# boundless-xyz/boundless

Hardware: AMD Instinct MI355X
Metric: segment-proofs/sec @ 2^20 cycles (higher is better)
Workload: dtype u32 (BabyBear Montgomery)

## Files before the change

### boundless_amd/csrc/poseidon2.hip

```cpp
#include "ctx.hpp"
#include "poseidon2_arith.hpp"
#include "hash_suite.hpp"
#include "../../include/bx_image.h"

namespace bx {

constexpr int CELLS = 24, RATE = 16, RF_HALF = 4, RP = 21;
constexpr int DIAG_OFF = 216;

__device__ __forceinline__ void poseidon2_mix(uint32_t* io, const uint32_t* __restrict__ prm) {
    i32 s[CELLS];
    i64 y[CELLS];
#pragma unroll
    for (int i = 0; i < CELLS; ++i) s[i] = (i32)io[i];
    m_ext64s(s, y);
    redc64s_all(y, prm, s);
#pragma unroll 1
    for (int r = 0; r < RF_HALF; ++r) {
        sbox7s_n<CELLS / 2>(s);
        sbox7s_n<CELLS / 2>(s + CELLS / 2);
        m_ext64s(s, y);
        if (r < RF_HALF - 1) {
            redc64s_all(y, prm + (r + 1) * CELLS, s);
        } else {
            red64ks_all<K1_MID, K2_MID, true>(y, prm[96], s);
        }
    }
    uint32_t diag[CELLS];
    {
        uint32_t zero;
        asm volatile("v_mov_b32 %0, 0" : "=v"(zero));
        const uint4* dp = reinterpret_cast<const uint4*>(prm + DIAG_OFF + zero);
#pragma unroll
        for (int i = 0; i < CELLS / 4; ++i) {
            const uint4 v = dp[i];
            diag[4 * i] = __builtin_amdgcn_readfirstlane(v.x);
            diag[4 * i + 1] = __builtin_amdgcn_readfirstlane(v.y);
            diag[4 * i + 2] = __builtin_amdgcn_readfirstlane(v.z);
            diag[4 * i + 3] = __builtin_amdgcn_readfirstlane(v.w);
        }
    }
#pragma unroll 1
    for (int r = 0; r < RP - 1; ++r) {
        internal_round<false>(s, diag, prm + 97 + r);
    }
    internal_round<true>(s, diag, prm + 117);
#pragma unroll 1
    for (int r = 0; r < RF_HALF; ++r) {
        sbox7s_n<CELLS / 2>(s);
        sbox7s_n<CELLS / 2>(s + CELLS / 2);
        m_ext64s(s, y);
        if (r < RF_HALF - 1) {
            redc64s_all(y, prm + 117 + (r + 1) * CELLS, s);
        } else {
            red64ks_all<K1_END, K2_END, false>(y, 0u, s);
#pragma unroll
            for (int i = 0; i < CELLS; ++i) io[i] = canon(s[i]);
        }
    }
}

__global__ __launch_bounds__(256) __attribute__((amdgpu_waves_per_eu(4, 4))) void hash_rows_kernel(uint32_t* __restrict__ out, const uint32_t* __restrict__ matrix,
                                                        const uint32_t* __restrict__ prm, uint32_t rows, uint32_t cols) {
    uint32_t r = blockIdx.x * blockDim.x + threadIdx.x;
    if (r >= rows) return;
    uint32_t s[CELLS];
#pragma unroll
    for (int i = 0; i < CELLS; ++i) s[i] = 0u;
    const uint32_t* p = matrix + r;
    uint32_t c = 0;
    for (; c + RATE <= cols; c += RATE) {
#pragma unroll
        for (int i = 0; i < RATE; ++i) s[i] = p[(size_t)(c + i) * rows];
        poseidon2_mix(s, prm);
    }
    if (c < cols || cols == 0) {
#pragma unroll
        for (int i = 0; i < RATE; ++i) s[i] = (c + i < cols) ? p[(size_t)(c + i) * rows] : 0u;
        poseidon2_mix(s, prm);
    }
    uint4* o = reinterpret_cast<uint4*>(out + (size_t)r * 8);
    o[0] = make_uint4(s[0], s[1], s[2], s[3]);
    o[1] = make_uint4(s[4], s[5], s[6], s[7]);
}

__global__ __launch_bounds__(256) __attribute__((amdgpu_waves_per_eu(4, 4))) void hash_fold_kernel(uint32_t* __restrict__ io, const uint32_t* __restrict__ prm,
                                                        uint32_t input_size, uint32_t output_size) {
    uint32_t i = blockIdx.x * blockDim.x + threadIdx.x;
    if (i >= output_size) return;
    const uint4* src = reinterpret_cast<const uint4*>(io + ((size_t)input_size + 2 * (size_t)i) * 8);
    uint32_t s[CELLS];
    uint4 v0 = src[0], v1 = src[1], v2 = src[2], v3 = src[3];
    s[0] = v0.x; s[1] = v0.y; s[2] = v0.z; s[3] = v0.w;
    s[4] = v1.x; s[5] = v1.y; s[6] = v1.z; s[7] = v1.w;
    s[8] = v2.x; s[9] = v2.y; s[10] = v2.z; s[11] = v2.w;
    s[12] = v3.x; s[13] = v3.y; s[14] = v3.z; s[15] = v3.w;
#pragma unroll
    for (int k = 16; k < CELLS; ++k) s[k] = 0u;
    poseidon2_mix(s, prm);
    uint4* o = reinterpret_cast<uint4*>(io + ((size_t)output_size + i) * 8);
    o[0] = make_uint4(s[0], s[1], s[2], s[3]);
    o[1] = make_uint4(s[4], s[5], s[6], s[7]);
}

__global__ __launch_bounds__(256) __attribute__((amdgpu_waves_per_eu(4, 4))) void hash_fold_indexed_kernel(uint32_t* out, const uint32_t* in,
                                                                const uint32_t* __restrict__ sel, const uint32_t* __restrict__ prm,
                                                                uint32_t count, uint32_t n_in) {
    uint32_t j = blockIdx.x * blockDim.x + threadIdx.x;
    if (j >= count) return;
    uint2 pr = reinterpret_cast<const uint2*>(sel)[j];
    pr.x = pr.x < n_in ? pr.x : n_in - 1;
    pr.y = pr.y < n_in ? pr.y : n_in - 1;
    const uint4* a = reinterpret_cast<const uint4*>(in + (size_t)pr.x * 8);
    const uint4* b = reinterpret_cast<const uint4*>(in + (size_t)pr.y * 8);
    uint32_t s[CELLS];
    uint4 v0 = a[0], v1 = a[1], v2 = b[0], v3 = b[1];
    s[0] = v0.x; s[1] = v0.y; s[2] = v0.z; s[3] = v0.w;
    s[4] = v1.x; s[5] = v1.y; s[6] = v1.z; s[7] = v1.w;
    s[8] = v2.x; s[9] = v2.y; s[10] = v2.z; s[11] = v2.w;
    s[12] = v3.x; s[13] = v3.y; s[14] = v3.z; s[15] = v3.w;
#pragma unroll
    for (int k = 16; k < CELLS; ++k) s[k] = 0u;
    poseidon2_mix(s, prm);
    uint4* o = reinterpret_cast<uint4*>(out + (size_t)j * 8);
    o[0] = make_uint4(s[0], s[1], s[2], s[3]);
    o[1] = make_uint4(s[4], s[5], s[6], s[7]);
}

__device__ __forceinline__ void fold_pair(uint32_t* out8, const uint32_t* a8, const uint32_t* b8, const uint32_t* __restrict__ prm) {
    uint32_t s[CELLS];
#pragma unroll
    for (int k = 0; k < 8; ++k) s[k] = a8[k], s[8 + k] = b8[k];
#pragma unroll
    for (int k = 16; k < CELLS; ++k) s[k] = 0u;
    poseidon2_mix(s, prm);
#pragma unroll
    for (int k = 0; k < 8; ++k) out8[k] = s[k];
}
__device__ __forceinline__ void ld_digest(uint32_t* d, const uint32_t* p) {
    const uint4 a = reinterpret_cast<const uint4*>(p)[0], b = reinterpret_cast<const uint4*>(p)[1];
    d[0] = a.x; d[1] = a.y; d[2] = a.z; d[3] = a.w; d[4] = b.x; d[5] = b.y; d[6] = b.z; d[7] = b.w;
}
__device__ __forceinline__ void st_digest(uint32_t* p, const uint32_t* d) {
    reinterpret_cast<uint4*>(p)[0] = make_uint4(d[0], d[1], d[2], d[3]);
    reinterpret_cast<uint4*>(p)[1] = make_uint4(d[4], d[5], d[6], d[7]);
}
template <int LVL>
__device__ __forceinline__ void fold_subtree(uint32_t* out8, uint32_t* __restrict__ io, const uint32_t* __restrict__ prm, size_t input_size, size_t idx) {
    uint32_t a[8], b[8];
    if constexpr (LVL == 1) {
        ld_digest(a, io + (input_size + 2 * idx) * 8);
        ld_digest(b, io + (input_size + 2 * idx + 1) * 8);
    } else {
        fold_subtree<LVL - 1>(a, io, prm, input_size, 2 * idx);
        fold_subtree<LVL - 1>(b, io, prm, input_size, 2 * idx + 1);
    }
    fold_pair(out8, a, b, prm);
    st_digest(io + ((input_size >> LVL) + idx) * 8, out8);
}
template <int L>
__global__ __launch_bounds__(256) __attribute__((amdgpu_waves_per_eu(4, 4))) void hash_fold_deep_kernel(uint32_t* __restrict__ io, const uint32_t* __restrict__ prm,
                                                                                               uint32_t input_size) {
    const uint32_t j = blockIdx.x * blockDim.x + threadIdx.x;
    if (j >= (input_size >> L)) return;
    uint32_t top[8];
    fold_subtree<L>(top, io, prm, input_size, j);
}

__global__ __launch_bounds__(256) __attribute__((amdgpu_waves_per_eu(4, 4))) void hash_fold_multi_kernel(uint32_t* __restrict__ io, const uint32_t* __restrict__ prm,
                                                              uint32_t input_size, uint32_t per_wg, int levels) {
    __shared__ uint32_t sh[256 * 8];
    const uint32_t tid = threadIdx.x;
    uint32_t width = per_wg >> 1;
    uint32_t out_size = input_size >> 1;
    uint32_t s[CELLS];
    if (tid < width) {
        const uint32_t i = blockIdx.x * width + tid;
        const uint4* src = reinterpret_cast<const uint4*>(io + ((size_t)input_size + 2 * (size_t)i) * 8);
        uint4 v0 = src[0], v1 = src[1], v2 = src[2], v3 = src[3];
        s[0] = v0.x; s[1] = v0.y; s[2] = v0.z; s[3] = v0.w;
        s[4] = v1.x; s[5] = v1.y; s[6] = v1.z; s[7] = v1.w;
        s[8] = v2.x; s[9] = v2.y; s[10] = v2.z; s[11] = v2.w;
        s[12] = v3.x; s[13] = v3.y; s[14] = v3.z; s[15] = v3.w;
#pragma unroll
        for (int k = 16; k < CELLS; ++k) s[k] = 0u;
        poseidon2_mix(s, prm);
        uint4* o = reinterpret_cast<uint4*>(io + ((size_t)out_size + i) * 8);
        o[0] = make_uint4(s[0], s[1], s[2], s[3]);
        o[1] = make_uint4(s[4], s[5], s[6], s[7]);
    }
    for (int lvl = 1; lvl < levels; ++lvl) {
        if (tid < width) {
#pragma unroll
            for (int k = 0; k < 8; ++k) sh[tid * 8 + k] = s[k];
        }
        __syncthreads();
        width >>= 1;
        out_size >>= 1;
        if (tid < width) {
#pragma unroll
            for (int k = 0; k < 16; ++k) s[k] = sh[tid * 16 + k];
#pragma unroll
            for (int k = 16; k < CELLS; ++k) s[k] = 0u;
            poseidon2_mix(s, prm);
            uint4* o = reinterpret_cast<uint4*>(io + ((size_t)out_size + blockIdx.x * width + tid) * 8);
            o[0] = make_uint4(s[0], s[1], s[2], s[3]);
            o[1] = make_uint4(s[4], s[5], s[6], s[7]);
        }
        __syncthreads();
    }
}

constexpr int QS = CELLS / 4;
__device__ __forceinline__ i32 quad_rot1(i32 v) { return __builtin_amdgcn_update_dpp(0, v, 0x39, 0xf, 0xf, false); }
__device__ __forceinline__ i32 quad_rot2(i32 v) { return __builtin_amdgcn_update_dpp(0, v, 0x4E, 0xf, 0xf, false); }
__device__ __forceinline__ i32 quad_rot3(i32 v) { return __builtin_amdgcn_update_dpp(0, v, 0x93, 0xf, 0xf, false); }
__device__ __forceinline__ i32 quad_xor1(i32 v) { return __builtin_amdgcn_update_dpp(0, v, 0xB1, 0xf, 0xf, false); }
__device__ __forceinline__ i64 add_u32v(i64 c, uint32_t k, int alt) {
#if defined(__HIP_DEVICE_COMPILE__)
    i64 r;
    BX_MAD_ASM("v_mad_u64_u32", "%1, 1, %2", "v"(k), "v"(c));
    return r;
#else
    (void)alt;
    return c + (i64)k;
#endif
}
struct QuadCoef {
    i32 c0, c1, c3;
};
__device__ __forceinline__ void m_ext_quad(const i32* s, i64* y, const QuadCoef& m) {
    i64 t = 0;
#pragma unroll
    for (int k = 0; k < QS; ++k) {
        const i32 x1 = quad_rot1(s[k]), x2 = quad_rot2(s[k]), x3 = quad_rot3(s[k]);
        i64 w = smul(s[k], m.c0, k);
        w = smad(x1, m.c1, w, k + 1);
        w = smadc<1>(x2, w, k + 2);
        w = smad(x3, m.c3, w, k + 3);
        y[k] = w;
        t += w;
    }
#pragma unroll
    for (int k = 0; k < QS; ++k) y[k] += t;
}
__device__ __forceinline__ void redc_quad(const i64* y, const uint32_t* __restrict__ rc , i32* s) {
    i64 acc[QS];
#pragma unroll
    for (int k = 0; k < QS; ++k) acc[k] = add_u32v(y[k], rc[4 * k], k);
    sredc_n<QS>(acc, s);
}
template <uint32_t K1, uint32_t K2>
__device__ __forceinline__ void redk_quad(const i64* y, uint32_t add0 , i32* s) {
    i64 acc[QS];
#pragma unroll
    for (int k = 0; k < QS; ++k) acc[k] = umul_k((uint32_t)y[k], K1, k);
    acc[0] = add_u32v(acc[0], add0, 0);
#pragma unroll
    for (int k = 0; k < QS; ++k) acc[k] = smad_k((i32)(y[k] >> 32), K2, acc[k], k + 1);
    sredc_n<QS>(acc, s);
}
template <bool RC_ALL>
__device__ __forceinline__ void internal_round_quad(i32* s, const i32* diag, uint32_t rc0 ,
                                                    const uint32_t* __restrict__ rc_all, uint32_t keep_mask) {
    const i32 sb = sbox7s(s[0]);
    s[0] = (i32)(((uint32_t)sb & keep_mask) | ((uint32_t)s[0] & ~keep_mask));
    i64 pa = smulc<1>(s[0], 0);
#pragma unroll
    for (int k = 1; k < QS; ++k) pa = smadc<1>(s[k], pa, k);
    {
        i64 o = (i64)(((uint64_t)(uint32_t)quad_xor1((i32)(pa >> 32)) << 32) | (uint32_t)quad_xor1((i32)(uint32_t)pa));
        pa += o;
        o = (i64)(((uint64_t)(uint32_t)quad_rot2((i32)(pa >> 32)) << 32) | (uint32_t)quad_rot2((i32)(uint32_t)pa));
        pa += o;
    }
    const i64 c = smulc<1>(internal_sum_rs(pa), 1);
    i64 tt[QS];
#pragma unroll
    for (int k = 0; k < QS; ++k) {
        if (RC_ALL) tt[k] = smad(s[k], diag[k], add_u32v(c, rc_all[4 * k], 2 * k), 2 * k + 1);
        else if (k == 0) tt[k] = smad(s[k], diag[k], add_u32v(c, rc0, 0), 1);
        else tt[k] = smad(s[k], diag[k], c, k + 1);
    }
    sredc_n<QS>(tt, s);
}
__device__ __forceinline__ void poseidon2_mix_quad(uint32_t* io, const uint32_t* __restrict__ shp, uint32_t q) {
    i32 s[QS];
    i64 y[QS];
    const bool odd = q & 1;
    const QuadCoef m{odd ? 6 : 5, odd ? 1 : 7, odd ? 4 : 3};
    const uint32_t keep = q == 0 ? 0xffffffffu : 0u;
#pragma unroll
    for (int k = 0; k < QS; ++k) s[k] = (i32)io[k];
    m_ext_quad(s, y, m);
    redc_quad(y, shp + q, s);
#pragma unroll 1
    for (int r = 0; r < RF_HALF; ++r) {
        sbox7s_n<QS>(s);
        m_ext_quad(s, y, m);
        if (r < RF_HALF - 1) redc_quad(y, shp + (r + 1) * CELLS + q, s);
        else redk_quad<K1_MID, K2_MID>(y, shp[96] & keep, s);
    }
    i32 diag[QS];
#pragma unroll
    for (int k = 0; k < QS; ++k) diag[k] = (i32)shp[DIAG_OFF + 4 * k + q];
#pragma unroll 1
    for (int r = 0; r < RP - 1; ++r) internal_round_quad<false>(s, diag, shp[97 + r] & keep, nullptr, keep);
    internal_round_quad<true>(s, diag, 0u, shp + 117 + q, keep);
#pragma unroll 1
    for (int r = 0; r < RF_HALF; ++r) {
        sbox7s_n<QS>(s);
        m_ext_quad(s, y, m);
        if (r < RF_HALF - 1) redc_quad(y, shp + 117 + (r + 1) * CELLS + q, s);
        else redk_quad<K1_END, K2_END>(y, 0u, s);
    }
#pragma unroll
    for (int k = 0; k < QS; ++k) io[k] = canon(s[k]);
}

__global__ __launch_bounds__(1024) void hash_fold_quad_kernel(uint32_t* __restrict__ io, const uint32_t* __restrict__ prm, uint32_t input_size,
                                                              uint32_t per_wg, int levels) {
    __shared__ uint32_t sh[256 * 8];
    __shared__ uint32_t shp[DIAG_OFF + 24];
    const uint32_t tid = threadIdx.x, q = tid & 3, node = tid >> 2;
    for (uint32_t i = tid; i < DIAG_OFF + 24; i += blockDim.x) shp[i] = prm[i];
    uint32_t width = per_wg >> 1;
    uint32_t out_size = input_size >> 1;
    for (int lvl = 0; lvl < levels; ++lvl) {
        const bool active = node < width;
        uint32_t s[QS];
        if (active) {
            if (lvl == 0) {
                const uint32_t* src = io + ((size_t)input_size + 2 * ((size_t)blockIdx.x * width + node)) * 8;
#pragma unroll
                for (int k = 0; k < 4; ++k) s[k] = src[4 * k + q];
            } else {
#pragma unroll
                for (int k = 0; k < 4; ++k) s[k] = sh[node * 16 + 4 * k + q];
            }
            s[4] = 0u;
            s[5] = 0u;
        }
        __syncthreads();
        if (active) {
            poseidon2_mix_quad(s, shp, q);
            uint32_t* o = io + ((size_t)out_size + (size_t)blockIdx.x * width + node) * 8;
            o[q] = s[0];
            o[4 + q] = s[1];
            sh[node * 8 + q] = s[0];
            sh[node * 8 + 4 + q] = s[1];
        }
        __syncthreads();
        width >>= 1;
        out_size >>= 1;
    }
}

__global__ __launch_bounds__(64) void transcript_step_kernel(uint32_t* __restrict__ state, const uint32_t* __restrict__ digests, uint32_t n_commit,
                                                            uint32_t* __restrict__ out, uint32_t n_elems, const uint32_t* __restrict__ prm) {
    __shared__ uint32_t shp[DIAG_OFF + 24];
    const uint32_t tid = threadIdx.x, q = tid & 3;
    for (uint32_t i = tid; i < DIAG_OFF + 24; i += blockDim.x) shp[i] = prm[i];
    __syncthreads();
    if (tid >= 4) return;
    uint32_t s[QS];
#pragma unroll
    for (int k = 0; k < QS; ++k) s[k] = state[4 * k + q];
    uint32_t pool = state[24];
    for (uint32_t i = 0; i < n_commit; ++i) {
        if (pool != 0) {
            poseidon2_mix_quad(s, shp, q);
            pool = 0;
        }
        s[0] = fp_add(s[0], digests[8 * i + q]);
        s[1] = fp_add(s[1], digests[8 * i + 4 + q]);
        poseidon2_mix_quad(s, shp, q);
    }
    for (uint32_t e = 0; e < n_elems; ++e) {
        if (pool == 16) {
            poseidon2_mix_quad(s, shp, q);
            pool = 0;
        }
        const uint32_t slot = pool >> 2;
        const uint32_t v = slot == 0 ? s[0] : slot == 1 ? s[1] : slot == 2 ? s[2] : s[3];
        if ((pool & 3u) == q) out[e] = v;
        ++pool;
    }
#pragma unroll
    for (int k = 0; k < QS; ++k) state[4 * k + q] = s[k];
    if (q == 0) state[24] = pool;
}

const char* poseidon2_upload_params(bx_ctx* c) {
    uint32_t h[DIAG_OFF + 24] = {0};
    for (int i = 0; i < 213; ++i) h[i] = (uint32_t)((uint64_t)(c->h_rc[i] % P) * p2_rc_scale(i) % P);
    for (int i = 0; i < 24; ++i) h[DIAG_OFF + i] = fp_encode(c->h_diag[i]);
    if (!c->d_p2) BX_HIP(c, hipMalloc(&c->d_p2, sizeof h));
    BX_HIP(c, hipMemcpyAsync(c->d_p2, h, sizeof h, hipMemcpyHostToDevice, c->stream));
    BX_HIP(c, stream_wait(c));
    return nullptr;
}

static const char* launch_hash_rows(bx_ctx* c, uint32_t* out, const uint32_t* matrix, size_t rows, size_t cols) {
    if (rows == 0) return nullptr;
    unsigned bs = (unsigned)c->hash_rows_block;
    hipLaunchKernelGGL(hash_rows_kernel, dim3((unsigned)((rows + bs - 1) / bs)), dim3(bs), 0, c->stream, out, matrix, c->d_p2,
                       (uint32_t)rows, (uint32_t)cols);
    BX_LAUNCH_CHECK(c);
    return nullptr;
}
static const char* launch_hash_fold(bx_ctx* c, uint32_t* io, size_t input_size, size_t output_size) {
    if (output_size == 0) return nullptr;
    hipLaunchKernelGGL(hash_fold_kernel, dim3((unsigned)((output_size + 255) / 256)), dim3(256), 0, c->stream, io, c->d_p2,
                       (uint32_t)input_size, (uint32_t)output_size);
    BX_LAUNCH_CHECK(c);
    return nullptr;
}
template <int L>
static const char* launch_hash_fold_deep(bx_ctx* c, uint32_t* io, size_t size) {
    hipLaunchKernelGGL(hash_fold_deep_kernel<L>, dim3((unsigned)(((size >> L) + 255) / 256)), dim3(256), 0, c->stream, io, c->d_p2, (uint32_t)size);
    BX_LAUNCH_CHECK(c);
    return nullptr;
}
static const char* launch_hash_fold_small(bx_ctx* c, uint32_t* io, size_t size, size_t per_wg, int levels) {
    if (c->fold_quad)
        hipLaunchKernelGGL(hash_fold_quad_kernel, dim3((unsigned)(size / per_wg)), dim3((unsigned)(2 * per_wg)), 0, c->stream, io, c->d_p2,
                           (uint32_t)size, (uint32_t)per_wg, levels);
    else
        hipLaunchKernelGGL(hash_fold_multi_kernel, dim3((unsigned)(size / per_wg)), dim3(256), 0, c->stream, io, c->d_p2, (uint32_t)size,
                           (uint32_t)per_wg, levels);
    BX_LAUNCH_CHECK(c);
    return nullptr;
}
HashLaunchers poseidon2_launchers() { return {launch_hash_rows, launch_hash_fold, launch_hash_fold_deep<3>, launch_hash_fold_deep<2>, launch_hash_fold_small}; }

}

using namespace bx;

extern "C" const char* bx_poseidon2_set_params(bx_ctx* c, const uint32_t* rc213, const uint32_t* diag24) try {
    if (!c) return "bx_poseidon2_set_params: null ctx";
    BX_REQUIRE(c, rc213 && diag24, "poseidon2_set_params: null table");
    BX_REQUIRE(c, c->live_provers == 0, "poseidon2_set_params: destroy the provers of this ctx first (their transcripts hold the old table)");
    BX_ENTER(c);
    for (int i = 0; i < 213; ++i) c->h_rc[i] = rc213[i] % P;
    for (int i = 0; i < 24; ++i) c->h_diag[i] = diag24[i] % P;
    return poseidon2_upload_params(c);
} BX_ABI_CATCH(c, "bx_poseidon2_set_params")
extern "C" const char* bx_poseidon2_get_params(bx_ctx* c, uint32_t* rc213, uint32_t* diag24) try {
    if (!c) return "bx_poseidon2_get_params: null ctx";
    for (int i = 0; i < 213; ++i) rc213[i] = c->h_rc[i];
    for (int i = 0; i < 24; ++i) diag24[i] = c->h_diag[i];
    return nullptr;
} BX_ABI_CATCH(c, "bx_poseidon2_get_params")

extern "C" const char* bx_hash_fold_indexed(bx_ctx* c, bx_buf out, bx_buf in, bx_buf sel, size_t count) try {
    if (!c) return "bx_hash_fold_indexed: null ctx";
    BX_REQUIRE(c, count <= out.len / 8 && count <= sel.len / 2, "hash_fold_indexed: out or sel too small");
    BX_REQUIRE(c, count <= 0xffffffffu && in.len / 8 <= 0xffffffffu, "hash_fold_indexed: too many digests");
    if (count == 0) return nullptr;
    BX_REQUIRE(c, out.dptr && in.dptr && sel.dptr && in.len >= 8, "hash_fold_indexed: null or empty buffer");
    BX_ENTER(c);
    OpScope op(c, "hash_fold_indexed", 104.0 * (double)count);
    hipLaunchKernelGGL(hash_fold_indexed_kernel, dim3((unsigned)((count + 255) / 256)), dim3(256), 0, c->stream, (uint32_t*)out.dptr,
                       (const uint32_t*)in.dptr, (const uint32_t*)sel.dptr, c->d_p2, (uint32_t)count, (uint32_t)(in.len / 8));
    BX_LAUNCH_CHECK(c);
    return nullptr;
} BX_ABI_CATCH(c, "bx_hash_fold_indexed")

extern "C" const char* bx_transcript_step(bx_ctx* c, bx_buf state, bx_buf digests, size_t n_commit, bx_buf out_ext, size_t n_ext) try {
    if (!c) return "bx_transcript_step: null ctx";
    BX_REQUIRE(c, c->hash_suite == SUITE_POSEIDON2, "transcript_step: the device transcript is Poseidon2's (a sha-256 ctx draws on the host)");
    BX_REQUIRE(c, state.dptr != nullptr && state.len >= 25, "transcript_step: the state is 24 cells and the pool counter");
    BX_REQUIRE(c, n_commit <= 64 && n_ext <= 64, "transcript_step: at most 64 commits and 64 challenges per step");
    BX_REQUIRE(c, digests.len >= 8 * n_commit && out_ext.len >= 4 * n_ext, "transcript_step: digests / out too small");
    BX_ENTER(c);
    if (!n_commit && !n_ext) return nullptr;
    OpScope op(c, "transcript_step", 4.0 * (double)(50 + 8 * n_commit + 4 * n_ext));
    hipLaunchKernelGGL(transcript_step_kernel, dim3(1), dim3(64), 0, c->stream, (uint32_t*)state.dptr, (const uint32_t*)digests.dptr, (uint32_t)n_commit,
                       (uint32_t*)out_ext.dptr, (uint32_t)(4 * n_ext), c->d_p2);
    BX_LAUNCH_CHECK(c);
    return nullptr;
} BX_ABI_CATCH(c, "bx_transcript_step")
```

### boundless_amd/csrc/poseidon2_arith.hpp

```cpp
#pragma once
#include "fp.hpp"

#if defined(BX_CHECK_BOUNDS) && !defined(__HIP_DEVICE_COMPILE__)
#include <stdio.h>
#include <stdlib.h>
#define BX_ASSERT_BOUND(cond, what)                                              \
    do {                                                                         \
        if (!(cond)) {                                                           \
            fprintf(stderr, "bound violated: %s (%s:%d)\n", what, __FILE__, __LINE__); \
            abort();                                                             \
        }                                                                        \
    } while (0)
#else
#define BX_ASSERT_BOUND(cond, what) ((void)0)
#endif

#if defined(BX_PLAIN_MAD)
#define BX_MAD_FLAVOUR mad_plain
#else
#define BX_MAD_FLAVOUR mad_pinned
#endif
namespace bx {
inline namespace BX_MAD_FLAVOUR {

constexpr int P2_CELLS = 24;

constexpr uint32_t cx_mul(uint32_t a, uint32_t b) { return (uint32_t)((uint64_t)a * b % P); }
constexpr uint32_t cx_pow(uint32_t b, uint64_t e) {
    uint32_t r = 1;
    while (e) {
        if (e & 1) r = cx_mul(r, b);
        b = cx_mul(b, b);
        e >>= 1;
    }
    return r;
}
constexpr uint32_t cx_rpow(int64_t e) { return cx_pow(MONT_ONE, e >= 0 ? (uint64_t)e : (uint64_t)((int64_t)(P - 1) + e)); }
constexpr uint32_t K1_MID = cx_rpow(2801), K2_MID = cx_mul(K1_MID, MONT_ONE);
constexpr uint32_t K1_END = cx_rpow(400), K2_END = cx_mul(K1_END, MONT_ONE);
constexpr uint32_t p2_rc_scale(int i) {
    return i < 24 ? cx_rpow(1) : i < 48 ? cx_rpow(-6) : i < 72 ? cx_rpow(-55) : i < 96 ? cx_rpow(-398)
         : i < 141 ? cx_rpow(2)
         : i < 165 ? cx_rpow(1) : i < 189 ? cx_rpow(-6) : cx_rpow(-55);
}

using i32 = int32_t;
using i64 = int64_t;
constexpr i64 SREDC_MAX = ((i64)0x7fffffff - (i64)(P / 2) - 2) * ((i64)1 << 32);

#if defined(__HIP_DEVICE_COMPILE__) && !defined(BX_PLAIN_MAD)
#define BX_MAD_ASM(op, args, ...)                                                                  \
    do {                                                                                           \
        switch (alt & 3) {                                                                         \
            case 0: asm volatile(op " %0, s[40:41], " args : "=v"(r) : __VA_ARGS__ : "s40", "s41"); break; \
            case 1: asm volatile(op " %0, s[42:43], " args : "=v"(r) : __VA_ARGS__ : "s42", "s43"); break; \
            case 2: asm volatile(op " %0, s[44:45], " args : "=v"(r) : __VA_ARGS__ : "s44", "s45"); break; \
            default: asm volatile(op " %0, s[46:47], " args : "=v"(r) : __VA_ARGS__ : "s46", "s47"); break; \
        }                                                                                          \
    } while (0)
#endif
BX_HD i64 smad(i32 a, i32 b, i64 c, int alt = 0) {
#if defined(__HIP_DEVICE_COMPILE__) && !defined(BX_PLAIN_MAD)
    i64 r;
    BX_MAD_ASM("v_mad_i64_i32", "%1, %2, %3", "v"(a), "v"(b), "v"(c));
    return r;
#else
    (void)alt;
    return (i64)a * (i64)b + c;
#endif
}
BX_HD i64 smul(i32 a, i32 b, int alt = 0) {
#if defined(__HIP_DEVICE_COMPILE__) && !defined(BX_PLAIN_MAD)
    i64 r;
    BX_MAD_ASM("v_mad_i64_i32", "%1, %2, 0", "v"(a), "v"(b));
    return r;
#else
    (void)alt;
    return (i64)a * (i64)b;
#endif
}
BX_HD i64 smad_k(i32 a, uint32_t k, i64 c, int alt = 0) {
#if defined(__HIP_DEVICE_COMPILE__) && !defined(BX_PLAIN_MAD)
    i64 r;
    BX_MAD_ASM("v_mad_i64_i32", "%1, %2, %3", "v"(a), "s"(k), "v"(c));
    return r;
#else
    (void)alt;
    return (i64)a * (i64)k + c;
#endif
}
BX_HD i64 smul_k(i32 a, uint32_t k, int alt = 0) {
#if defined(__HIP_DEVICE_COMPILE__) && !defined(BX_PLAIN_MAD)
    i64 r;
    BX_MAD_ASM("v_mad_i64_i32", "%1, %2, 0", "v"(a), "s"(k));
    return r;
#else
    (void)alt;
    return (i64)a * (i64)k;
#endif
}
template <int K>
BX_HD i64 smadc(i32 a, i64 c, int alt = 0) {
#if defined(__HIP_DEVICE_COMPILE__) && !defined(BX_PLAIN_MAD)
    i64 r;
    BX_MAD_ASM("v_mad_i64_i32", "%1, %3, %2", "v"(a), "v"(c), "n"(K));
    return r;
#else
    (void)alt;
    return (i64)a * K + c;
#endif
}
template <int K>
BX_HD i64 smulc(i32 a, int alt = 0) {
#if defined(__HIP_DEVICE_COMPILE__) && !defined(BX_PLAIN_MAD)
    i64 r;
    BX_MAD_ASM("v_mad_i64_i32", "%1, %2, 0", "v"(a), "n"(K));
    return r;
#else
    (void)alt;
    return (i64)a * K;
#endif
}
BX_HD i64 add_u32(i64 c, uint32_t k, int alt = 0) {
#if defined(__HIP_DEVICE_COMPILE__) && !defined(BX_PLAIN_MAD)
    i64 r;
    BX_MAD_ASM("v_mad_u64_u32", "%1, 1, %2", "s"(k), "v"(c));
    return r;
#else
    (void)alt;
    return c + (i64)k;
#endif
}
BX_HD i64 umul_k(uint32_t a, uint32_t k, int alt = 0) {
#if defined(__HIP_DEVICE_COMPILE__) && !defined(BX_PLAIN_MAD)
    i64 r;
    BX_MAD_ASM("v_mad_u64_u32", "%1, %2, 0", "v"(a), "s"(k));
    return r;
#else
    (void)alt;
    return (i64)((uint64_t)a * (uint64_t)k);
#endif
}
BX_HD i32 mont_m(i64 t) {
#if defined(__HIP_DEVICE_COMPILE__) && !defined(BX_PLAIN_MAD)
    i32 m;
    asm volatile("v_mul_lo_u32 %0, %1, %2" : "=v"(m) : "v"((uint32_t)t), "s"(NEG_P_INV));
    return m;
#else
    return (i32)((uint32_t)t * NEG_P_INV);
#endif
}
BX_HD i32 sredc(i64 t, int alt = 0) {
    BX_ASSERT_BOUND(t <= SREDC_MAX && t >= -SREDC_MAX, "sredc operand");
    const i32 m = mont_m(t);
    return (i32)(smad_k(m, P, t, alt) >> 32);
}
BX_HD i64 iabs64(i64 v) { return v < 0 ? -v : v; }

constexpr i64 ub(i64 T) { return (T >> 32) + (i64)(P / 2) + 1; }
constexpr i64 B_IN = (i64)P - 1;
constexpr i64 B_Y = 112 * ((i64)1 << 31);
constexpr i64 B_EXT = ub(B_Y + (i64)P);
constexpr i64 B_MIDOUT = ub(((i64)1 << 32) * K1_MID + ((B_Y >> 32) + 1) * (i64)K2_MID + 2 * (i64)P);
constexpr i64 B_SUMR = ub(((i64)1 << 31) * R2 + 33 * (i64)R3);
constexpr i64 B_INT = (i64)((double)P * 0.945);
static_assert(ub((i64)(P - 1) * B_INT + B_SUMR + (i64)P) <= B_INT && B_MIDOUT <= B_INT, "internal-round bound is not invariant");
static_assert((i64)(P - 1) * B_INT + B_SUMR + (i64)P <= SREDC_MAX && B_INT * B_INT <= SREDC_MAX, "internal-round products overflow sredc");
static_assert(24 * B_INT < ((i64)1 << 37), "internal sum");

BX_HD uint64_t mad64(uint32_t a, uint32_t b, uint64_t c) { return (uint64_t)a * (uint64_t)b + c; }

template <int N>
BX_HD void sredc_n(const i64* t, i32* r) {
    i32 m[N];
#pragma unroll
    for (int i = 0; i < N; ++i) {
        BX_ASSERT_BOUND(t[i] <= SREDC_MAX && t[i] >= -SREDC_MAX, "sredc operand");
        m[i] = mont_m(t[i]);
    }
#pragma unroll
    for (int i = 0; i < N; ++i) r[i] = (i32)(smad_k(m[i], P, t[i], i & 3) >> 32);
}

BX_HD i32 sbox7s(i32 x) {
    BX_ASSERT_BOUND(iabs64(x) <= B_INT, "sbox input");
    const i32 x2 = sredc(smul(x, x));
    const i32 x3 = sredc(smul(x2, x));
    const i32 x4 = sredc(smul(x2, x2));
    return sredc(smul(x3, x4));
}
template <int N>
BX_HD void sbox7s_n(i32* x) {
    i64 t[N], u[N];
    i32 x2[N], x3[N], x4[N];
#pragma unroll
    for (int i = 0; i < N; ++i) {
        BX_ASSERT_BOUND(iabs64(x[i]) <= B_INT, "sbox input");
        t[i] = smul(x[i], x[i], i & 3);
    }
    sredc_n<N>(t, x2);
#pragma unroll
    for (int i = 0; i < N; ++i) {
        t[i] = smul(x2[i], x[i], 2 * i);
        u[i] = smul(x2[i], x2[i], 2 * i + 1);
    }
    sredc_n<N>(t, x3);
    sredc_n<N>(u, x4);
#pragma unroll
    for (int i = 0; i < N; ++i) t[i] = smul(x3[i], x4[i], i & 3);
    sredc_n<N>(t, x);
}

BX_HD i32 redc64s(i64 y, uint32_t rc) {
    BX_ASSERT_BOUND(iabs64(y) <= B_Y, "external layer output");
    const i32 r = sredc(add_u32(y, rc));
    BX_ASSERT_BOUND(iabs64(r) <= B_EXT, "redc64s output");
    return r;
}

BX_HD void redc64s_all(const i64* y, const uint32_t* rc, i32* s) {
    constexpr int H = P2_CELLS / 2;
#pragma unroll
    for (int h = 0; h < P2_CELLS; h += H) {
        i64 acc[H];
#pragma unroll
        for (int i = 0; i < H; ++i) {
            BX_ASSERT_BOUND(iabs64(y[h + i]) <= B_Y, "external layer output");
            acc[i] = add_u32(y[h + i], rc[h + i], i & 3);
        }
        sredc_n<H>(acc, s + h);
    }
#pragma unroll
    for (int i = 0; i < P2_CELLS; ++i) BX_ASSERT_BOUND(iabs64(s[i]) <= B_EXT, "redc64s output");
}

template <uint32_t K1, uint32_t K2, bool HAS_ADD = true>
BX_HD i32 red64ks(i64 y, uint32_t add) {
    BX_ASSERT_BOUND(iabs64(y) <= B_Y, "external layer output");
    static_assert(K1 < (1u << 29) && K2 < P, "correction constant too large for the accumulator bound");
    i64 acc = umul_k((uint32_t)y, K1);
    if (HAS_ADD) acc = add_u32(acc, add);
    return sredc(smad_k((i32)(y >> 32), K2, acc));
}
template <uint32_t K1, uint32_t K2, bool HAS_ADD0>
BX_HD void red64ks_all(const i64* y, uint32_t add0, i32* s) {
    static_assert(K1 < (1u << 29) && K2 < P, "correction constant too large for the accumulator bound");
    constexpr int H = P2_CELLS / 2;
#pragma unroll
    for (int h = 0; h < P2_CELLS; h += H) {
        i64 acc[H];
#pragma unroll
        for (int i = 0; i < H; ++i) {
            BX_ASSERT_BOUND(iabs64(y[h + i]) <= B_Y, "external layer output");
            acc[i] = umul_k((uint32_t)y[h + i], K1, i & 3);
        }
        if (HAS_ADD0 && h == 0) acc[0] = add_u32(acc[0], add0, 0);
#pragma unroll
        for (int i = 0; i < H; ++i) acc[i] = smad_k((i32)(y[h + i] >> 32), K2, acc[i], (i + 1) & 3);
        sredc_n<H>(acc, s + h);
    }
}

BX_HD void m_ext64s(const i32* s, i64* y) {
#pragma unroll
    for (int h = 0; h < 2; ++h) {
        i64 t0[3], t1[3], t2[3], t3[3];
#pragma unroll
        for (int q = 0; q < 3; ++q) {
            const int g = 3 * h + q;
            t0[q] = smulc<1>(s[4 * g], 2 * q);
            t1[q] = smulc<1>(s[4 * g + 2], 2 * q + 1);
        }
#pragma unroll
        for (int q = 0; q < 3; ++q) {
            const int g = 3 * h + q;
            t0[q] = smadc<1>(s[4 * g + 1], t0[q], 2 * q + 2);
            t1[q] = smadc<1>(s[4 * g + 3], t1[q], 2 * q + 3);
        }
#pragma unroll
        for (int q = 0; q < 3; ++q) {
            const int g = 3 * h + q;
            t2[q] = smadc<2>(s[4 * g + 1], t1[q], 2 * q);
            t3[q] = smadc<2>(s[4 * g + 3], t0[q], 2 * q + 1);
        }
#pragma unroll
        for (int q = 0; q < 3; ++q) {
            const int g = 3 * h + q;
            const i64 t4 = t1[q] * 4 + t3[q], t5 = t0[q] * 4 + t2[q];
            y[4 * g] = t3[q] + t5;
            y[4 * g + 1] = t5;
            y[4 * g + 2] = t2[q] + t4;
            y[4 * g + 3] = t4;
        }
    }
    i64 t[4];
#pragma unroll
    for (int j = 0; j < 4; ++j) {
        t[j] = y[j];
#pragma unroll
        for (int k = 4; k < P2_CELLS; k += 4) t[j] += y[k + j];
    }
#pragma unroll
    for (int i = 0; i < P2_CELLS; ++i) y[i] += t[i & 3];
}

BX_HD i32 internal_sum_rs(i64 sum) {
    BX_ASSERT_BOUND(iabs64(sum) < ((i64)1 << 37), "internal sum < 2^37");
    const i32 lo = (i32)(uint32_t)sum;
    const i32 hi = (i32)(sum >> 32) - (lo >> 31);
    const i32 r = sredc(smad_k(hi, R3, smul_k(lo, R2)));
    BX_ASSERT_BOUND(iabs64(r) <= B_SUMR, "sum_r");
    return r;
}
template <bool RC_ALL>
BX_HD void internal_round(i32* s, const uint32_t* diag, const uint32_t* rc) {
    BX_ASSERT_BOUND(iabs64(s[0]) <= B_INT, "sbox input");
    i64 pa = smulc<1>(s[1], 0), pb = smulc<1>(s[2], 1);
    i64 t = smul(s[0], s[0], 2);
    pa = smadc<1>(s[3], pa, 3);
    i32 m = mont_m(t);
    pb = smadc<1>(s[4], pb, 0);
    const i32 x2 = (i32)(smad_k(m, P, t, 1) >> 32);
    pa = smadc<1>(s[5], pa, 2);
    t = smul(x2, s[0], 3);
    pb = smadc<1>(s[6], pb, 0);
    i64 u = smul(x2, x2, 1);
    pa = smadc<1>(s[7], pa, 2);
    m = mont_m(t);
    pb = smadc<1>(s[8], pb, 3);
    i32 m2 = mont_m(u);
    pa = smadc<1>(s[9], pa, 0);
    const i32 x3 = (i32)(smad_k(m, P, t, 1) >> 32);
    pb = smadc<1>(s[10], pb, 2);
    const i32 x4 = (i32)(smad_k(m2, P, u, 3) >> 32);
    pa = smadc<1>(s[11], pa, 0);
    t = smul(x3, x4, 1);
    pb = smadc<1>(s[12], pb, 2);
    pa = smadc<1>(s[13], pa, 3);
    m = mont_m(t);
    pb = smadc<1>(s[14], pb, 0);
    pa = smadc<1>(s[15], pa, 1);
    s[0] = (i32)(smad_k(m, P, t, 2) >> 32);
#pragma unroll
    for (int i = 16; i < P2_CELLS; ++i) {
        if (i & 1) pa = smadc<1>(s[i], pa, i + 3);
        else pb = smadc<1>(s[i], pb, i + 3);
    }
    pa = smadc<1>(s[0], pa, 3);
    const i64 sum = pa + pb;
    const i64 c = smulc<1>(internal_sum_rs(sum), 1);
    constexpr int H = P2_CELLS / 2;
#pragma unroll
    for (int h = 0; h < P2_CELLS; h += H) {
        i64 tt[H];
#pragma unroll
        for (int i = 0; i < H; ++i) {
            if (RC_ALL || h + i == 0)
                tt[i] = smad_k(s[h + i], diag[h + i], add_u32(c, rc[h + i], 2 * i + 2), 2 * i + 3);
            else
                tt[i] = smad_k(s[h + i], diag[h + i], c, i + 2);
        }
        sredc_n<H>(tt, s + h);
    }
#pragma unroll
    for (int i = 0; i < P2_CELLS; ++i) BX_ASSERT_BOUND(iabs64(s[i]) <= B_INT, "internal cell");
}

BX_HD i32 fp_centre(uint32_t v) { return (i32)v - (v > P / 2 ? (i32)P : 0); }
BX_HD uint32_t canon(i32 v) {
    BX_ASSERT_BOUND(iabs64(v) < (i64)P, "canonicalisation input");
    const uint32_t u = (uint32_t)v;
    return umin(u, u + P);
}

template <int DIAG>
BX_HD void poseidon2_mix_bounded(uint32_t* io, const uint32_t* prm) {
    i32 s[P2_CELLS];
    i64 y[P2_CELLS];
    const uint32_t* diag = prm + DIAG;
    for (int i = 0; i < P2_CELLS; ++i) {
        BX_ASSERT_BOUND(io[i] <= B_IN, "canonical input");
        s[i] = (i32)io[i];
    }
    m_ext64s(s, y);
    redc64s_all(y, prm, s);
    for (int r = 0; r < 4; ++r) {
        sbox7s_n<P2_CELLS>(s);
        m_ext64s(s, y);
        if (r < 3) {
            redc64s_all(y, prm + (r + 1) * P2_CELLS, s);
        } else {
            red64ks_all<K1_MID, K2_MID, true>(y, prm[96], s);
            for (int i = 0; i < P2_CELLS; ++i) BX_ASSERT_BOUND(iabs64(s[i]) <= B_MIDOUT, "mid transition output");
        }
    }
    for (int r = 0; r < 20; ++r) internal_round<false>(s, diag, prm + 97 + r);
    internal_round<true>(s, diag, prm + 117);
    for (int r = 0; r < 4; ++r) {
        sbox7s_n<P2_CELLS>(s);
        m_ext64s(s, y);
        if (r < 3) {
            redc64s_all(y, prm + 117 + (r + 1) * P2_CELLS, s);
        } else {
            red64ks_all<K1_END, K2_END, false>(y, 0u, s);
            for (int i = 0; i < P2_CELLS; ++i) io[i] = canon(s[i]);
        }
    }
}

}
}
```

Before: 28.03.

## Fuse pairs of Poseidon2 internal rounds into one algebraic step

Replaces the 20 single internal rounds with 10 paired rounds. Each pair uses precomputed diag² and diag·R² constants uploaded after the diag table, so the second round's full-state reduction is folded into the first's and the two rounds' dot products are interleaved with the S-box chains. This is meant to cut per-cell Montgomery reductions and expose more instruction-level parallelism. In exchange it needs careful 64-bit bound proofs (static_asserts), more scalar constants and more register pressure.

```diff
diff --git a/boundless_amd/csrc/poseidon2.hip b/boundless_amd/csrc/poseidon2.hip
--- a/boundless_amd/csrc/poseidon2.hip
+++ b/boundless_amd/csrc/poseidon2.hip
@@ -7,6 +7,7 @@
 
 constexpr int CELLS = 24, RATE = 16, RF_HALF = 4, RP = 21;
 constexpr int DIAG_OFF = 216;
+constexpr int PAIR_OFF = DIAG_OFF + 24, P2_TABLE = PAIR_OFF + 2 * CELLS;
 
 __device__ __forceinline__ void poseidon2_mix(uint32_t* io, const uint32_t* __restrict__ prm) {
     i32 s[CELLS];
@@ -26,10 +27,26 @@
             red64ks_all<K1_MID, K2_MID, true>(y, prm[96], s);
         }
     }
+    uint32_t zero;
+    asm volatile("v_mov_b32 %0, 0" : "=v"(zero));
+    {
+        i32 pk[2 * CELLS];
+        const uint4* kp = reinterpret_cast<const uint4*>(prm + PAIR_OFF + zero);
+#pragma unroll
+        for (int i = 0; i < 2 * CELLS / 4; ++i) {
+            const uint4 v = kp[i];
+            pk[4 * i] = (i32)__builtin_amdgcn_readfirstlane(v.x);
+            pk[4 * i + 1] = (i32)__builtin_amdgcn_readfirstlane(v.y);
+            pk[4 * i + 2] = (i32)__builtin_amdgcn_readfirstlane(v.z);
+            pk[4 * i + 3] = (i32)__builtin_amdgcn_readfirstlane(v.w);
+        }
+#pragma unroll 1
+        for (int r = 0; r < RP - 1; r += 2) {
+            internal_round_pair(s, pk, pk + CELLS, prm + 97 + r);
+        }
+    }
     uint32_t diag[CELLS];
     {
-        uint32_t zero;
-        asm volatile("v_mov_b32 %0, 0" : "=v"(zero));
         const uint4* dp = reinterpret_cast<const uint4*>(prm + DIAG_OFF + zero);
 #pragma unroll
         for (int i = 0; i < CELLS / 4; ++i) {
@@ -39,10 +56,6 @@
             diag[4 * i + 2] = __builtin_amdgcn_readfirstlane(v.z);
             diag[4 * i + 3] = __builtin_amdgcn_readfirstlane(v.w);
         }
-    }
-#pragma unroll 1
-    for (int r = 0; r < RP - 1; ++r) {
-        internal_round<false>(s, diag, prm + 97 + r);
     }
     internal_round<true>(s, diag, prm + 117);
 #pragma unroll 1
@@ -133,7 +146,9 @@
     for (int k = 0; k < 8; ++k) s[k] = a8[k], s[8 + k] = b8[k];
 #pragma unroll
     for (int k = 16; k < CELLS; ++k) s[k] = 0u;
-    poseidon2_mix(s, prm);
+    uint32_t z;
+    asm volatile("s_mov_b32 %0, 0" : "=s"(z));
+    poseidon2_mix(s, prm + z);
 #pragma unroll
     for (int k = 0; k < 8; ++k) out8[k] = s[k];
 }
@@ -392,9 +407,12 @@
 }
 
 const char* poseidon2_upload_params(bx_ctx* c) {
-    uint32_t h[DIAG_OFF + 24] = {0};
+    uint32_t h[P2_TABLE] = {0};
     for (int i = 0; i < 213; ++i) h[i] = (uint32_t)((uint64_t)(c->h_rc[i] % P) * p2_rc_scale(i) % P);
     for (int i = 0; i < 24; ++i) h[DIAG_OFF + i] = fp_encode(c->h_diag[i]);
+    i32 pe[CELLS], pa[CELLS];
+    p2_pair_consts(h + DIAG_OFF, pe, pa);
+    for (int i = 0; i < CELLS; ++i) h[PAIR_OFF + i] = (uint32_t)pe[i], h[PAIR_OFF + CELLS + i] = (uint32_t)pa[i];
     if (!c->d_p2) BX_HIP(c, hipMalloc(&c->d_p2, sizeof h));
     BX_HIP(c, hipMemcpyAsync(c->d_p2, h, sizeof h, hipMemcpyHostToDevice, c->stream));
     BX_HIP(c, stream_wait(c));
diff --git a/boundless_amd/csrc/poseidon2_arith.hpp b/boundless_amd/csrc/poseidon2_arith.hpp
--- a/boundless_amd/csrc/poseidon2_arith.hpp
+++ b/boundless_amd/csrc/poseidon2_arith.hpp
@@ -90,6 +90,26 @@
 #endif
 }
 BX_HD i64 smul_k(i32 a, uint32_t k, int alt = 0) {
+#if defined(__HIP_DEVICE_COMPILE__) && !defined(BX_PLAIN_MAD)
+    i64 r;
+    BX_MAD_ASM("v_mad_i64_i32", "%1, %2, 0", "v"(a), "s"(k));
+    return r;
+#else
+    (void)alt;
+    return (i64)a * (i64)k;
+#endif
+}
+BX_HD i64 smad_s(i32 a, i32 k, i64 c, int alt = 0) {
+#if defined(__HIP_DEVICE_COMPILE__) && !defined(BX_PLAIN_MAD)
+    i64 r;
+    BX_MAD_ASM("v_mad_i64_i32", "%1, %2, %3", "v"(a), "s"(k), "v"(c));
+    return r;
+#else
+    (void)alt;
+    return (i64)a * (i64)k + c;
+#endif
+}
+BX_HD i64 smul_s(i32 a, i32 k, int alt = 0) {
 #if defined(__HIP_DEVICE_COMPILE__) && !defined(BX_PLAIN_MAD)
     i64 r;
     BX_MAD_ASM("v_mad_i64_i32", "%1, %2, 0", "v"(a), "s"(k));
@@ -367,6 +387,145 @@
 }
 
 BX_HD i32 fp_centre(uint32_t v) { return (i32)v - (v > P / 2 ? (i32)P : 0); }
+
+constexpr i64 fold_ub(i64 T) { return ((T >> 32) + 1) * (i64)MONT_ONE + ((i64)1 << 32); }
+constexpr i64 B_K = (i64)(P / 2);
+constexpr i64 B_SBOX = ub(ub(ub(B_INT * B_INT) * B_INT) * ub(ub(B_INT * B_INT) * ub(B_INT * B_INT)));
+constexpr i64 B_SIG1 = ub(fold_ub((i64)1 << 37));
+constexpr i64 T_DOT = 4 * B_K * B_INT + B_K * B_SIG1;
+static_assert(T_DOT <= INT64_MAX && fold_ub(T_DOT) + 4 * B_K * B_INT <= T_DOT, "dot-product group overflows 64 bits");
+constexpr i64 T_LAST = 2 * fold_ub(T_DOT) + 3 * B_K * B_INT + B_SBOX * (i64)R2;
+static_assert(T_LAST <= INT64_MAX && fold_ub(T_LAST) <= SREDC_MAX, "last dot-product group overflows");
+constexpr i64 B_SIG2 = ub(fold_ub(T_LAST));
+constexpr i64 T_PAIR0 = B_K * B_SBOX + B_SIG1 * (i64)R2 + (i64)P;
+constexpr i64 T_PAIRI = B_K * B_INT + B_K * B_SIG1 + B_SIG2;
+static_assert(B_SIG2 <= B_SIG1 * (i64)R2 && T_PAIR0 <= SREDC_MAX && ub(T_PAIR0) <= B_INT, "paired rounds: cell 0 leaves the internal-round bound");
+static_assert(T_PAIRI <= SREDC_MAX && ub(T_PAIRI) <= B_INT, "paired rounds: cells 1..23 leave the internal-round bound");
+constexpr i32 K23R3 = (i32)cx_mul(23u, R3) - (cx_mul(23u, R3) > P / 2 ? (i32)P : 0);
+
+BX_HD i64 fold64(i64 g, int alt = 0) { return smad_k((i32)(g >> 32), MONT_ONE, (i64)(uint32_t)g, alt); }
+BX_HD void p2_pair_consts(const uint32_t* diag, i32* E, i32* A) {
+    E[0] = fp_centre(diag[0]);
+    A[0] = 0;
+    for (int i = 1; i < P2_CELLS; ++i) {
+        E[i] = fp_centre(fp_mul(diag[i], diag[i]));
+        A[i] = fp_centre(fp_mul(diag[i], R2));
+    }
+}
+BX_HD void internal_round_pair(i32* s, const i32* E, const i32* A, const uint32_t* rc) {
+    BX_ASSERT_BOUND(iabs64(s[0]) <= B_INT, "sbox input");
+    i64 pa = smulc<1>(s[1], 0), pb = smulc<1>(s[2], 1);
+    i64 t = smul(s[0], s[0], 2);
+    pa = smadc<1>(s[3], pa, 3);
+    i32 m = mont_m(t);
+    pb = smadc<1>(s[4], pb, 0);
+    i32 x2 = (i32)(smad_k(m, P, t, 1) >> 32);
+    pa = smadc<1>(s[5], pa, 2);
+    t = smul(x2, s[0], 3);
+    pb = smadc<1>(s[6], pb, 0);
+    i64 u = smul(x2, x2, 1);
+    pa = smadc<1>(s[7], pa, 2);
+    m = mont_m(t);
+    pb = smadc<1>(s[8], pb, 3);
+    i32 m2 = mont_m(u);
+    pa = smadc<1>(s[9], pa, 0);
+    i32 x3 = (i32)(smad_k(m, P, t, 1) >> 32);
+    pb = smadc<1>(s[10], pb, 2);
+    i32 x4 = (i32)(smad_k(m2, P, u, 3) >> 32);
+    pa = smadc<1>(s[11], pa, 0);
+    t = smul(x3, x4, 1);
+    pb = smadc<1>(s[12], pb, 2);
+    pa = smadc<1>(s[13], pa, 3);
+    m = mont_m(t);
+    pb = smadc<1>(s[14], pb, 0);
+    pa = smadc<1>(s[15], pa, 1);
+    const i32 x0 = (i32)(smad_k(m, P, t, 2) >> 32);
+#pragma unroll
+    for (int i = 16; i < P2_CELLS; ++i) {
+        if (i & 1) pa = smadc<1>(s[i], pa, i + 3);
+        else pb = smadc<1>(s[i], pb, i + 3);
+    }
+    pa = smadc<1>(x0, pa, 3);
+    i64 gx = smul_s(s[1], A[1], 0), gy = smul_s(s[5], A[5], 1);
+    const i64 sum1 = pa + pb;
+    BX_ASSERT_BOUND(iabs64(sum1) < ((i64)1 << 37) && iabs64(x0) <= B_SBOX, "internal sum < 2^37");
+    i64 a0 = smul_s(x0, E[0], 2);
+    i64 f = fold64(sum1, 3);
+    gx = smad_s(s[2], A[2], gx, 0);
+    m = mont_m(f);
+    gy = smad_s(s[6], A[6], gy, 1);
+    const i32 sig1 = (i32)(smad_k(m, P, f, 2) >> 32);
+    BX_ASSERT_BOUND(iabs64(sig1) <= B_SIG1, "sig1");
+    gx = smad_s(s[3], A[3], gx, 3);
+    gy = smad_s(s[7], A[7], gy, 0);
+    a0 = smad_k(sig1, R2, a0, 1);
+    gx = smad_s(s[4], A[4], gx, 2);
+    a0 = add_u32(a0, rc[0], 3);
+    BX_ASSERT_BOUND(iabs64(a0) <= T_PAIR0, "cell 0, round A");
+    gy = smad_s(s[8], A[8], gy, 0);
+    m = mont_m(a0);
+    gx = smad_s(sig1, K23R3, gx, 1);
+    const i32 y0 = (i32)(smad_k(m, P, a0, 2) >> 32);
+    BX_ASSERT_BOUND(iabs64(y0) <= B_INT && iabs64(gx) <= T_DOT && iabs64(gy) <= T_DOT, "sbox input");
+    i64 fx = fold64(gx, 3);
+    t = smul(y0, y0, 0);
+    i64 fy = fold64(gy, 1);
+    gx = smad_s(s[9], A[9], fx, 2);
+    m = mont_m(t);
+    gy = smad_s(s[13], A[13], fy, 3);
+    x2 = (i32)(smad_k(m, P, t, 0) >> 32);
+    gx = smad_s(s[10], A[10], gx, 1);
+    gy = smad_s(s[14], A[14], gy, 2);
+    t = smul(x2, y0, 3);
+    gx = smad_s(s[11], A[11], gx, 0);
+    u = smul(x2, x2, 1);
+    gy = smad_s(s[15], A[15], gy, 2);
+    m = mont_m(t);
+    gx = smad_s(s[12], A[12], gx, 3);
+    m2 = mont_m(u);
+    gy = smad_s(s[16], A[16], gy, 0);
+    x3 = (i32)(smad_k(m, P, t, 1) >> 32);
+    BX_ASSERT_BOUND(iabs64(gx) <= T_DOT && iabs64(gy) <= T_DOT, "dot-product group");
+    fx = fold64(gx, 2);
+    x4 = (i32)(smad_k(m2, P, u, 3) >> 32);
+    fy = fold64(gy, 0);
+    t = smul(x3, x4, 1);
+    gx = smad_s(s[17], A[17], fx, 2);
+    gx = smad_s(s[18], A[18], gx, 3);
+    m = mont_m(t);
+    gx = smad_s(s[19], A[19], gx, 0);
+    gx = smad_s(s[20], A[20], gx, 1);
+    const i32 y0s = (i32)(smad_k(m, P, t, 2) >> 32);
+    BX_ASSERT_BOUND(iabs64(gx) <= T_DOT && iabs64(y0s) <= B_SBOX, "dot-product group");
+    fx = fold64(gx, 3);
+    gy = smad_s(s[21], A[21], fy, 0);
+    gy = smad_s(s[22], A[22], gy, 1);
+    gy = smad_s(s[23], A[23], gy, 2);
+    gy = smad_k(y0s, R2, gy + fx, 3);
+    BX_ASSERT_BOUND(iabs64(gy) <= T_LAST, "last dot-product group");
+    const i32 sig2 = sredc(fold64(gy, 0), 1);
+    BX_ASSERT_BOUND(iabs64(sig2) <= B_SIG2, "sig2");
+    const i64 c = smulc<1>(sig2, 2);
+    constexpr int H = P2_CELLS / 2;
+#pragma unroll
+    for (int h = 0; h < P2_CELLS; h += H) {
+        i64 tt[H];
+#pragma unroll
+        for (int i = 0; i < H; ++i) {
+            if (h + i == 0)
+                tt[i] = smad_s(y0s, E[0], add_u32(c, rc[1], 2), 3);
+            else
+                tt[i] = smad_s(s[h + i], E[h + i], c, i + 2);
+        }
+#pragma unroll
+        for (int i = 0; i < H; ++i)
+            if (h + i != 0) tt[i] = smad_s(sig1, A[h + i], tt[i], i + 1);
+        sredc_n<H>(tt, s + h);
+    }
+#pragma unroll
+    for (int i = 0; i < P2_CELLS; ++i) BX_ASSERT_BOUND(iabs64(s[i]) <= B_INT, "internal cell");
+}
+
 BX_HD uint32_t canon(i32 v) {
     BX_ASSERT_BOUND(iabs64(v) < (i64)P, "canonicalisation input");
     const uint32_t u = (uint32_t)v;
@@ -394,7 +553,9 @@
             for (int i = 0; i < P2_CELLS; ++i) BX_ASSERT_BOUND(iabs64(s[i]) <= B_MIDOUT, "mid transition output");
         }
     }
-    for (int r = 0; r < 20; ++r) internal_round<false>(s, diag, prm + 97 + r);
+    i32 pair_e[P2_CELLS], pair_a[P2_CELLS];
+    p2_pair_consts(diag, pair_e, pair_a);
+    for (int r = 0; r < 20; r += 2) internal_round_pair(s, pair_e, pair_a, prm + 97 + r);
     internal_round<true>(s, diag, prm + 117);
     for (int r = 0; r < 4; ++r) {
         sbox7s_n<P2_CELLS>(s);
```

Measured after the change: 28.87 (median of 6 runs). 3.0% higher.
